# ramkp990/Truth_Recommendation_GNN

Hardware: AMD Instinct MI355X
Metric: edges/s (fwd+bwd) hetero message-passing (higher is better)
Workload: dtype f32; 1 GPU; cfg4: U=9000000 P=1000000 E_engage=200000000 (+reverse), relations=rev_engages+engages, d=h=128, 2-layer hetero-SAGE train step (fwd+loss+bwd+Adam); global_batch=800000000, parallelism=single

## Files before the change

### include/hgnn.h

```cpp
#ifndef HGNN_H_
#define HGNN_H_

#include <stddef.h>
#include <stdint.h>

#ifdef __cplusplus
extern "C" {
#endif

#define HGNN_OK 0
#define HGNN_E_ARG 1001
#define HGNN_E_HIP 1002
#define HGNN_E_WS 1003
#define HGNN_E_UNSUPPORTED 1004

#define HGNN_MEAN 1
#define HGNN_ACCUMULATE 2

#define HGNN_MAX_SEG 6

typedef void* hgnn_stream_t;

int hgnn_version(void);
const char* hgnn_last_error_string(void);
// ... 198 lines not shown

int hgnn_gather_reduce_bf16(const uint16_t* x, int64_t n_x, int32_t d, const int32_t* rowptr,
                            const int32_t* col, int64_t n_rows, const float* edge_w,
                            const float* col_w, const float* row_w, int32_t flags,
                            const int32_t* heavy_rows, const int32_t* heavy_first,
                            int64_t n_heavy, int64_t n_chunks, int32_t chunk, float* slab,
                            float* out, int64_t acc_limit, const int32_t* col_hot,
                            float hot_share, hgnn_stream_t stream);

int hgnn_score_gather2_bf16(const uint16_t* x, int64_t n_x, const uint16_t* rowvec, int32_t d,
                            const int32_t* rowptr, const int32_t* col, const int32_t* rowptr_n,
                            const int32_t* col_n, int64_t n_rows, const float* cscale,
                            float inv_e, const int32_t* heavy_rows, const int32_t* heavy_first,
                            int64_t n_heavy, int64_t n_chunks, int32_t chunk, float* slab,
                            float* out, hgnn_stream_t stream);

int hgnn_edge_score_fwd_bf16(const uint16_t* U, const uint16_t* P, int32_t d, int64_t n_users,
                             int64_t n_posts, const int32_t* rowptr_u, const int32_t* col_u,
                             const int64_t* neg_i64, const int32_t* neg_i32,
                             const uint64_t* d_seed, int64_t n_edges, const float* cscale,
                             float* dU, float* part, float* loss, int32_t* err,
                             hgnn_stream_t stream);

size_t hgnn_sample_ws_bytes(int64_t n_dst);
int hgnn_sample_neighbors(const int32_t* rowptr, const int32_t* col, int64_t n_rows,
                          const int32_t* dst_ids, int64_t n_dst, int32_t fanout, uint64_t seed,
                          int32_t* out_rowptr, int32_t* out_col, void* ws, size_t ws_bytes,
                          hgnn_stream_t stream);
int hgnn_sample_fill(const int32_t* rowptr, const int32_t* col, int64_t n_rows,
                     const int32_t* dst_ids, int64_t n_dst, int32_t fanout, uint64_t seed,
                     const int32_t* out_rowptr, int32_t* out_col, hgnn_stream_t stream);
size_t hgnn_sample_hop_ws_bytes(int64_t n_total_dst);
int hgnn_sample_hop_count(int32_t n_rel, const int32_t* const* rowptrs, const int64_t* n_rows,
                          const int32_t* const* dst_ids, const int64_t* n_dst, int32_t fanout,
                          int32_t* const* out_rowptrs, int32_t* d_totals, void* ws,
                          size_t ws_bytes, hgnn_stream_t stream);
int hgnn_sample_hop_fill(int32_t n_rel, const int32_t* const* rowptrs, const int32_t* const* cols,
                         const int64_t* n_rows, const int32_t* const* dst_ids,
                         const int64_t* n_dst, int32_t fanout, uint64_t seed,
                         const int32_t* const* out_rowptrs, int32_t* const* out_cols,
                         hgnn_stream_t stream);

size_t hgnn_relabel_ws_bytes(int64_t n_prefix, int64_t n_items);
int hgnn_relabel(const int32_t* prefix, int64_t n_prefix, const int32_t* items, int64_t n_items,
                 int32_t* local_out, int32_t* nodes_out, int32_t* d_count, void* ws,
                 size_t ws_bytes, hgnn_stream_t stream);
// ... 98 lines not shown
```

### truth_recommendation_gnn_amd/_native.py

```python
from __future__ import annotations

import ctypes
import os
import pathlib
from typing import Optional, Sequence

import torch

LIB_PATH = pathlib.Path(__file__).resolve().parent / "lib" / "libhgnn.so"
if os.environ.get("HGNN_LIB"):
    LIB_PATH = LIB_PATH.parent / pathlib.Path(os.environ["HGNN_LIB"]).name

HGNN_MEAN = 1
HGNN_ACCUMULATE = 2
MAX_SEG = 6

_c_i32, _c_i64, _c_sz, _p = ctypes.c_int32, ctypes.c_int64, ctypes.c_size_t, ctypes.c_void_p

_SIGS = {
    "hgnn_version": (_c_i32, []),
    "hgnn_last_error_string": (ctypes.c_char_p, []),
    "hgnn_coo_to_csr_ws_bytes": (_c_sz, [_c_i64, _c_i64]),
    "hgnn_coo_to_csr": (_c_i32, [_p, _p, _c_i64, _c_i64, _c_i64, _p, _p, _p, _p, _p, _c_sz, _p]),
    "hgnn_plan_ws_bytes": (_c_sz, [_c_i64]),
# ... 95 lines not shown
    "hgnn_score_topk": (_c_i32, [_p, _p, _c_i64, _p, _c_i64, _c_i32, _c_i32, _p, _p, _p]),
    "hgnn_score_topk_bf16_lds_bytes": (_c_sz, [_c_i32, _c_i32]),
    "hgnn_score_topk_bf16": (_c_i32, [_p, _p, _c_i64, _p, _c_i64, _c_i32, _c_i32, _p, _p, _p]),
    "hgnn_score_topk_excl": (_c_i32, [_p, _p, _c_i64, _p, _c_i64, _c_i32, _c_i32, _p, _p, _p, _p,
                                      _p, _p]),
    "hgnn_score_topk_excl_bf16": (_c_i32, [_p, _p, _c_i64, _p, _c_i64, _c_i32, _c_i32, _p, _p,
                                           _p, _p, _p, _p]),
    "hgnn_topk_finish": (_c_i32, [_p, _p, _c_i64, _c_i32, _c_i64, _c_i32, _p, _p, _p, _p, _p, _p,
                                  _p]),
    "hgnn_edge_score_parts": (_c_i64, [_c_i64]),
    "hgnn_edge_score_fwd": (_c_i32, [_p, _p, _c_i32, _c_i64, _c_i64, _p, _p, _p, _p, _c_i64, _p,
                                     _p, _p, _p, _p, _p, _p, _p, _p, _p]),
    "hgnn_edge_score_fwd_i32": (_c_i32, [_p, _p, _c_i32, _c_i64, _c_i64, _p, _p, _p, _c_i64, _p,
                                         _p, _p, _p, _p, _p]),
    "hgnn_edge_score_fwd_draw": (_c_i32, [_p, _p, _c_i32, _c_i64, _c_i64, _p, _p, _p, _c_i64,
                                          _p, _p, _p, _p, _p, _p]),
    "hgnn_rows_to_bf16": (_c_i32, [_p, _c_i64, _p, _p]),
    "hgnn_gather_reduce_bf16": (_c_i32, [_p, _c_i64, _c_i32, _p, _p, _c_i64, _p, _p, _p, _c_i32,
                                         _p, _p, _c_i64, _c_i64, _c_i32, _p, _p, _c_i64, _p,
                                         ctypes.c_float, _p]),
    "hgnn_score_gather2_bf16": (_c_i32, [_p, _c_i64, _p, _c_i32, _p, _p, _p, _p, _c_i64, _p,
                                         ctypes.c_float, _p, _p, _c_i64, _c_i64, _c_i32, _p, _p,
                                         _p]),
    "hgnn_edge_score_fwd_bf16": (_c_i32, [_p, _p, _c_i32, _c_i64, _c_i64, _p, _p, _p, _p, _p,
                                          _c_i64, _p, _p, _p, _p, _p, _p]),
    "hgnn_uniform_i32": (_c_i32, [_p, _c_i64, _c_i32, _p, _p]),
    "hgnn_scale_unless_one": (_c_i32, [_p, _c_i64, _p, _p]),
    "hgnn_linear_fwd_f32": (_c_i32, [_p, _c_i64, _c_i32, _p, _c_i32, _p, _p, _p]),
    "hgnn_linear_dgrad_f32": (_c_i32, [_p, _c_i64, _c_i32, _p, _c_i32, _p, _p]),
    "hgnn_linear_wgrad_f32": (_c_i32, [_p, _p, _c_i64, _c_i32, _c_i32, _p, _p, _p, _c_sz, _p]),
    "hgnn_hetero_epilogue": (_c_i32, [_c_i32, _p, _p, _c_i64, _c_i32, _p, _p]),
    "hgnn_hetero_epilogue_bwd": (_c_i32, [_c_i32, _p, _c_i64, _c_i32, _p, _p, _p, _p]),
    "hgnn_idmap_capacity": (_c_i64, [_c_i64]),
    "hgnn_idmap_build": (_c_i32, [_p, _p, _p, _c_i64, _p, _c_i64, _p]),
    "hgnn_idmap_lookup": (_c_i32, [_p, _c_i64, _p, _p, _p, _p, _p, _p, _p, _p, _c_i64, _p, _p]),
    "hgnn_compact_rows_ws_bytes": (_c_sz, [_c_i64]),
    "hgnn_compact_rows": (_c_i32, [_p, _c_i32, _c_i64, _p, _p, _c_i32, _p, _p, _c_sz, _p]),
}

_lib: Optional[ctypes.CDLL] = None


class NativeError(RuntimeError):
    pass


# ... 94 lines not shown
```

### truth_recommendation_gnn_amd/build.py

```python
from __future__ import annotations

import concurrent.futures as cf
import hashlib
import json
import os
import pathlib
import subprocess
import sys

PKG = pathlib.Path(__file__).resolve().parent
CSRC = PKG / "csrc"
LIBDIR = PKG / "lib"
LIB = LIBDIR / "libhgnn.so"
INCLUDE = PKG.parent / "include"
HIPCC = os.environ.get("HIPCC", "/opt/rocm/bin/hipcc")
ARCH = "gfx950"
FLAGS = ["-O3", "-std=c++17", "-fPIC", f"--offload-arch={ARCH}", "-Wall",
         "-Wno-unused-result", f"-I{INCLUDE}"]
FILE_FLAGS = {"linear_xs": ["-fno-slp-vectorize"]}


def _sources():
    return sorted(CSRC.glob("*.hip"))


def _digest(extra=(), only=None) -> str:
    h = hashlib.sha256()
    for p in _sources() + sorted(CSRC.glob("*.h")) + [INCLUDE / "hgnn.h"]:
        h.update(p.name.encode())
        h.update(p.read_bytes())
    h.update(" ".join(f for f in FLAGS if not f.startswith("-I")).encode())
    h.update(repr(sorted(FILE_FLAGS.items())).encode())
    if extra:
        h.update(repr((list(extra), sorted(only) if only else None)).encode())
    return h.hexdigest()[:16]


def stamp_path(lib: pathlib.Path) -> pathlib.Path:
    return lib.with_name(lib.name[:-len(".so")] + ".digest")


def check_library(lib: pathlib.Path) -> None:
# ... 51 lines not shown
```

### truth_recommendation_gnn_amd/csrc/gather.hip

```cpp
#include "hgnn_common.h"

#include <stdlib.h>
#include <string.h>

namespace hgnn {

struct GatherArgs {
  const void* x;
  const int32_t* rowptr;
  const int32_t* col;
  const float* edge_w;
  const float* col_w;
  const float* row_w;
  const int32_t* heavy_rows;
  const int32_t* heavy_first;
  float* slab;
  float* out;
  int64_t n_rows;
  int64_t n_heavy;
  int64_t n_items;
  int32_t d;
  int32_t chunk;
  int32_t mean;
  int32_t accumulate;
  int64_t acc_limit;
  const void* rowvec;
  const float* cscale;
  float inv_e;
  int32_t score;
  const int32_t* rowptr2;
  int32_t nt_load;
  int32_t nt_store;
  const int32_t* col2;
  int32_t hot;
  int32_t bf16;
};

constexpr int32_t kHotIdMask = 0x7fffffff;

template <int LPR, int VPL, int W, int UNROLL, bool HAS_W, bool SC, bool HOT, typename XT = float>
__device__ __forceinline__ void segment_sum(const GatherArgs& a, const int32_t* col, int score,
                                            int64_t beg, int64_t end,
                                            const typename Vec<W>::T (&rv)[VPL],
                                            typename Vec<W>::T (&acc)[VPL]) {
  using V = Vec<W>;
  using S = RowSrc<XT, W>;
  constexpr int NS = 64 / LPR;
  const int lane = threadIdx.x & 63;
  const int slot = lane / LPR, sl = lane % LPR;
  const int d = a.d;
  for (int64_t base = beg; base < end; base += 64) {
    const int n = (int)min<int64_t>(64, end - base);
    int cidx = 0;
    float wv = 1.f;
    if (lane < n) {
      cidx = col[base + lane];
      if (HAS_W) {
        wv = a.edge_w ? a.edge_w[base + lane] : 1.f;
        if (a.col_w) wv *= a.col_w[HOT ? cidx & kHotIdMask : cidx];
      }
    }
    for (int j = 0; j < n; j += NS * UNROLL) {
      typename S::Raw v[UNROLL][VPL];
      float we[UNROLL];
#pragma unroll
      for (int u = 0; u < UNROLL; ++u) {
        const int e = j + u * NS + slot;
        const int raw = __shfl(cidx, e & 63, 64);
        const int src = HOT ? raw & kHotIdMask : raw;
// ... 24 lines not shown
        }
      }
#pragma unroll
      for (int u = 0; u < UNROLL; ++u)
#pragma unroll
        for (int q = 0; q < VPL; ++q) {
          if (HAS_W || SC) V::fma(acc[q], we[u], S::widen(v[u][q]));
          else V::add(acc[q], S::widen(v[u][q]));
        }
    }
  }
}

template <int LPR, int VPL, int W>
__device__ __forceinline__ void slot_combine(typename Vec<W>::T (&acc)[VPL]) {
  using V = Vec<W>;
#pragma unroll
  for (int m = LPR; m < 64; m <<= 1)
#pragma unroll
    for (int q = 0; q < VPL; ++q) V::add(acc[q], V::shfl_xor(acc[q], m));
}

template <int LPR, int VPL, int W, int UNROLL, bool HAS_W, bool SC, bool HOT = false,
          typename XT = float>
__device__ __forceinline__ void gather_item(const GatherArgs& a, const int64_t item) {
  using V = Vec<W>;
  using S = RowSrc<XT, W>;
  const int lane = threadIdx.x & 63;
  const int sl = lane % LPR;
  const bool writer = lane < LPR;
  int64_t row, beg, end;
  float* dst;
  bool partial;
  const bool two = SC && a.rowptr2;
  bool own = true;
  if (item < a.n_rows) {
    row = item;
    beg = a.rowptr[row];
    end = a.rowptr[row + 1];
    if (end - beg > a.chunk) {
      if (!two) return;
      own = false;
    }
    dst = a.out + row * a.d;
    partial = false;
  } else {
    const int64_t slot = item - a.n_rows;
    int64_t lo = 0, hi = a.n_heavy;
    while (hi - lo > 1) {
      int64_t mid = (lo + hi) >> 1;
      if (a.heavy_first[mid] <= slot) lo = mid; else hi = mid;
    }
    row = a.heavy_rows[lo];
    const int64_t k = slot - a.heavy_first[lo];
    beg = a.rowptr[row] + k * a.chunk;
    end = min<int64_t>(beg + a.chunk, a.rowptr[row + 1]);
    dst = a.slab + slot * a.d;
    partial = true;
  }
  typename V::T acc[VPL], rv[VPL];
#pragma unroll
  for (int q = 0; q < VPL; ++q) {
    acc[q] = V::zero();
    const int c = (q * LPR + sl) * W;
    rv[q] = (SC && c < a.d)
                ? S::widen(S::load(static_cast<const XT*>(a.rowvec) + row * a.d + c))
                : V::zero();
  }
  if (own)
    segment_sum<LPR, VPL, W, UNROLL, HAS_W, SC, HOT, XT>(a, a.col, a.score, beg, end, rv, acc);
  if (two && !partial)
    segment_sum<LPR, VPL, W, UNROLL, HAS_W, SC, false, XT>(a, a.col2, 2, a.rowptr2[row],
                                                           a.rowptr2[row + 1], rv, acc);
  slot_combine<LPR, VPL, W>(acc);
  if (!writer) return;
  float s = 1.f;
  if (!partial) {
    if (a.row_w) s = a.row_w[row];
    else if (a.mean) s = end > beg ? 1.f / (float)(end - beg) : 0.f;
  }
#pragma unroll
  for (int q = 0; q < VPL; ++q) {
    const int c = (q * LPR + sl) * W;
    if (c < a.d) {
      typename V::T r = acc[q];
      if (!partial) {
        V::scale(r, s);
        if (a.accumulate && (a.acc_limit == 0 || row < a.acc_limit)) V::add(r, V::load(dst + c));
      }
      if (a.nt_store) V::store_nt(dst + c, r);
      else V::store(dst + c, r);
    }
  }
}

template <int LPR, int VPL, int W, int UNROLL, bool HAS_W, bool SC = false, bool HOT = false,
          typename XT = float>
__global__ void __launch_bounds__(256) k_gather(const GatherArgs a) {
  const int64_t item = (int64_t)blockIdx.x * 4 + (threadIdx.x >> 6);
  if (item >= a.n_items) return;
  gather_item<LPR, VPL, W, UNROLL, HAS_W, SC, HOT, XT>(a, item);
}

constexpr int kGatherMultiMax = 8;
struct GatherMulti {
  GatherArgs j[kGatherMultiMax];
  int64_t base[kGatherMultiMax + 1];
  int32_t n;
};

template <int LPR, int VPL, int W, int UNROLL, bool HAS_W>
__global__ void __launch_bounds__(256) k_gather_multi(const GatherMulti m) {
  const int64_t item = (int64_t)blockIdx.x * 4 + __builtin_amdgcn_readfirstlane(threadIdx.x >> 6);
  if (item >= m.base[m.n]) return;
  int j = 0;
  while (j + 1 < m.n && item >= m.base[j + 1]) ++j;
  gather_item<LPR, VPL, W, UNROLL, HAS_W, false>(m.j[j], item - m.base[j]);
}

template <int W>
__global__ void __launch_bounds__(256) k_fixup(const GatherArgs a) {
  using V = Vec<W>;
  __shared__ typename V::T buf[256];
  const int64_t h = blockIdx.x;
// ... 40 lines not shown
    }
    __syncthreads();
  }
}

template <int LPR, int VPL, int W, int UNROLL>
static int launch_gather(const GatherArgs& a, bool has_w, hipStream_t stream) {
  const dim3 grid((unsigned)cdiv(a.n_items, 4)), block(256);
  if (a.score)
    hipLaunchKernelGGL((k_gather<LPR, VPL, W, UNROLL, false, true>), grid, block, 0, stream, a);
  else if (a.hot && has_w)
    hipLaunchKernelGGL((k_gather<LPR, VPL, W, UNROLL, true, false, true>), grid, block, 0, stream,
                       a);
  else if (a.hot)
    hipLaunchKernelGGL((k_gather<LPR, VPL, W, UNROLL, false, false, true>), grid, block, 0,
                       stream, a);
  else if (has_w)
    hipLaunchKernelGGL((k_gather<LPR, VPL, W, UNROLL, true>), grid, block, 0, stream, a);
  else
    hipLaunchKernelGGL((k_gather<LPR, VPL, W, UNROLL, false>), grid, block, 0, stream, a);
  return check_launch("k_gather");
}

static int dispatch_gather(const GatherArgs& a, bool has_w, hipStream_t stream) {
  const int d = a.d;
  if (d % 4 == 0) {
    const int nv = d / 4;
    if (nv <= 4) return launch_gather<4, 1, 4, 4>(a, has_w, stream);
    if (nv <= 8) return launch_gather<8, 1, 4, 4>(a, has_w, stream);
    if (nv <= 16) {
      const dim3 grid((unsigned)cdiv(a.n_items, 4)), block(256);
      if (a.score)
        hipLaunchKernelGGL((k_gather<16, 1, 4, 4, false, true>), grid, block, 0, stream, a);
      else if (a.hot && has_w)
        hipLaunchKernelGGL((k_gather<16, 1, 4, 6, true, false, true>), grid, block, 0, stream, a);
      else if (a.hot)
        hipLaunchKernelGGL((k_gather<16, 1, 4, 8, false, false, true>), grid, block, 0, stream, a);
      else if (has_w)
        hipLaunchKernelGGL((k_gather<16, 1, 4, 6, true>), grid, block, 0, stream, a);
      else
        hipLaunchKernelGGL((k_gather<16, 1, 4, 8, false>), grid, block, 0, stream, a);
      return check_launch("k_gather");
    }
    if (nv <= 32) return launch_gather<32, 1, 4, 4>(a, has_w, stream);
    if (nv <= 64) return launch_gather<64, 1, 4, 4>(a, has_w, stream);
    if (nv <= 128) return launch_gather<64, 2, 4, 2>(a, has_w, stream);
    if (nv <= 256) return launch_gather<64, 4, 4, 2>(a, has_w, stream);
    return fail(HGNN_E_UNSUPPORTED, "gather: d=%d > 1024", d);
// ... 256 lines not shown
  a.rowvec = rowvec; a.cscale = cscale; a.inv_e = inv_e; a.score = mode;
  nt_policy(a, n_x);
  return run_gather(a, as_stream(stream));
}

int hgnn_score_gather2(const float* x, int64_t n_x, const float* rowvec, int32_t d,
                       const int32_t* rowptr, const int32_t* col, const int32_t* rowptr_n,
                       const int32_t* col_n, int64_t n_rows, const float* cscale, float inv_e,
                       const int32_t* heavy_rows, const int32_t* heavy_first, int64_t n_heavy,
                       int64_t n_chunks, int32_t chunk, float* slab, float* out,
                       hgnn_stream_t stream) {
  if (!rowptr_n && n_rows > 0) return fail(HGNN_E_ARG, "score_gather2: rowptr_n is null");
  GatherArgs a{};
  a.x = x; a.rowptr = rowptr; a.col = col;
  a.heavy_rows = heavy_rows; a.heavy_first = heavy_first; a.slab = slab; a.out = out;
  a.n_rows = n_rows; a.n_heavy = n_heavy; a.n_items = n_rows + (n_heavy > 0 ? n_chunks : 0);
  a.d = d; a.chunk = chunk;
  a.rowvec = rowvec; a.cscale = cscale; a.inv_e = inv_e; a.score = 1;
  a.rowptr2 = rowptr_n; a.col2 = col_n;
  nt_policy(a, n_x);
  return run_gather(a, as_stream(stream));
}

int hgnn_score_gather2_bf16(const uint16_t* x, int64_t n_x, const uint16_t* rowvec, int32_t d,
                            const int32_t* rowptr, const int32_t* col, const int32_t* rowptr_n,
                            const int32_t* col_n, int64_t n_rows, const float* cscale,
                            float inv_e, const int32_t* heavy_rows, const int32_t* heavy_first,
                            int64_t n_heavy, int64_t n_chunks, int32_t chunk, float* slab,
                            float* out, hgnn_stream_t stream) {
  if (d > 0 && (d % 8 != 0 || d > 1024))
    return fail(HGNN_E_UNSUPPORTED,
                "score_gather2_bf16: d=%d (bf16 rows need d %% 8 == 0 and d <= 1024)", d);
  if (!rowptr_n && n_rows > 0) return fail(HGNN_E_ARG, "score_gather2_bf16: rowptr_n is null");
  GatherArgs a{};
  a.x = x; a.rowptr = rowptr; a.col = col;
  a.heavy_rows = heavy_rows; a.heavy_first = heavy_first; a.slab = slab; a.out = out;
  a.n_rows = n_rows; a.n_heavy = n_heavy; a.n_items = n_rows + (n_heavy > 0 ? n_chunks : 0);
  a.d = d; a.chunk = chunk;
  a.rowvec = rowvec; a.cscale = cscale; a.inv_e = inv_e; a.score = 1;
  a.rowptr2 = rowptr_n; a.col2 = col_n;
  a.bf16 = 1;
  nt_policy(a, n_x, 2);
  return run_gather(a, as_stream(stream));
}

}
// ... 1 lines not shown
```

### truth_recommendation_gnn_amd/ops.py

```python
from __future__ import annotations

import dataclasses
import os
import weakref
from typing import Dict, List, NamedTuple, Optional, Sequence, Tuple

import torch

from . import _native as N
from .graph import RelationCSR


def _check_f32(t: torch.Tensor, what: str) -> torch.Tensor:
    if t.dtype != torch.float32:
        raise TypeError(f"{what}: hgnn computes in fp32 (the reference dtype); got {t.dtype}")
    return t.contiguous()


ROW_DTYPES = ("fp32", "bf16")


def _row_dtype_value(v: str, what: str) -> str:
    if v not in ROW_DTYPES:
        raise ValueError(f"{what}={v!r}: the row storage is 'fp32' or 'bf16'")
# ... 297 lines not shown
        for i, (x, csr) in enumerate(pairs):
            if i < len(static) and static[i]:
                res[i] = gather_mean(x, csr, static=True,
                                     name=names[i] if i < len(names) else None)
            else:
                rest.append(i)
        if rest:
            for i, o in zip(rest, gather_mean_many([pairs[i] for i in rest])):
                res[i] = o
        return res
    jobs = []
    for x, csr in pairs:
        x = _check_f32(x, "gather_mean")
        if x.shape[0] != csr.n_src:
            raise ValueError(f"x_src has {x.shape[0]} rows, relation expects {csr.n_src}")
        if csr.num_edges and gather_blocks(x, csr.num_edges) > 1:
            return [gather_mean(x, c) for x, c in pairs]
        jobs.append((x, csr.fwd, torch.empty(csr.n_dst, int(x.shape[1]), dtype=torch.float32,
                                             device=x.device)))
    if not _multi_ok(jobs):
        return [gather_mean(x, c) for x, c in pairs]
    _gather_multi(jobs, mean=True, accumulate=False)
    return [o for _, _, o in jobs]


def _table_bytes(x: torch.Tensor) -> int:
    return x.numel() * x.element_size()


def _gather(x, grouped, col_w, csr_mean, out, accumulate, edge_w=None, kind=None, hot=None):
    p = grouped.plan
    dev = out.device
    slab = None
    if p.n_heavy:
        slab = torch.empty(p.n_chunks * out.shape[1], dtype=torch.float32, device=dev)
    flags = (N.HGNN_MEAN if csr_mean else 0) | (N.HGNN_ACCUMULATE if accumulate else 0)
    d = int(out.shape[1])
    weighted = edge_w is not None or col_w is not None
    kind = kind or ("fwd" if csr_mean else "bwd")
    name = f"gather_{kind}[{grouped.n_rows}<-{x.shape[0]}]x{d}"
    E = int(grouped.col.numel())
    rb = _row_bytes(x)
    with _timed(name, gather_bytes(E, grouped.n_rows, d, weighted, rb),
                gather_compulsory_bytes(E, grouped.n_rows, int(x.shape[0]), d, weighted, rb)):
        if x.dtype == torch.bfloat16:
            N.check(N.lib().hgnn_gather_reduce_bf16(
# ... 17 lines not shown
            N.ptr(p.heavy_first), p.n_heavy, p.n_chunks, p.chunk, N.ptr(slab), N.ptr(out),
            N.stream_ptr(dev)), "hgnn_gather_reduce")


def _score_gather(U, P, grouped, mode, cscale, inv_e, out, accumulate, tag):
    p = grouped.plan
    dev = out.device
    d = int(out.shape[1])
    slab = None
    if p.n_heavy:
        slab = torch.empty(p.n_chunks * d, dtype=torch.float32, device=dev)
    E = int(grouped.col.numel())
    nb = gather_bytes(E, grouped.n_rows, d, False) + 4 * grouped.n_rows * d
    cb = (gather_compulsory_bytes(E, grouped.n_rows, int(U.shape[0]), d, False)
          + 4 * grouped.n_rows * d)
    with _timed(f"score_gather_{tag}[{grouped.n_rows}<-{U.shape[0]}]x{d}", nb, cb):
        N.check(N.lib().hgnn_score_gather(
            N.ptr(U), U.shape[0], N.ptr(P), d, N.ptr(grouped.rowptr), N.ptr(grouped.col),
            grouped.n_rows, mode, N.ptr(cscale), inv_e, N.ptr(p.heavy_rows), N.ptr(p.heavy_first),
            p.n_heavy, p.n_chunks, p.chunk, N.ptr(slab), N.ptr(out), 1 if accumulate else 0,
            N.stream_ptr(dev)), "hgnn_score_gather")


def _score_gather2(U, P, pos, negs, cscale, inv_e, out):
    p = pos.plan
    dev = out.device
    d = int(out.shape[1])
    n = pos.n_rows
    slab = None
    if p.n_heavy:
        slab = torch.empty(p.n_chunks * d, dtype=torch.float32, device=dev)
    E = int(pos.col.numel()) + int(negs.col.numel())
    rb = _row_bytes(U)
    nb = gather_bytes(E, n, d, False, rb) + 4 * (n + 1) + n * rb
    cb = gather_compulsory_bytes(E, n, int(U.shape[0]), d, False, rb) + 4 * (n + 1) + n * rb
    with _timed(f"score_gather[{n}<-{U.shape[0]}]x{d}", nb, cb):
        if U.dtype == torch.bfloat16:
            N.check(N.lib().hgnn_score_gather2_bf16(
                N.ptr(U), U.shape[0], N.ptr(P), d, N.ptr(pos.rowptr), N.ptr(pos.col),
                N.ptr(negs.rowptr), N.ptr(negs.col), n, N.ptr(cscale), inv_e,
                N.ptr(p.heavy_rows), N.ptr(p.heavy_first), p.n_heavy, p.n_chunks, p.chunk,
                N.ptr(slab), N.ptr(out), N.stream_ptr(dev)), "hgnn_score_gather2_bf16")
            return
        N.check(N.lib().hgnn_score_gather2(
            N.ptr(U), U.shape[0], N.ptr(P), d, N.ptr(pos.rowptr), N.ptr(pos.col),
            N.ptr(negs.rowptr), N.ptr(negs.col), n, N.ptr(cscale), inv_e, N.ptr(p.heavy_rows),
            N.ptr(p.heavy_first), p.n_heavy, p.n_chunks, p.chunk, N.ptr(slab), N.ptr(out),
            N.stream_ptr(dev)), "hgnn_score_gather2")


def scatter_mean_bwd(grad_aggr: torch.Tensor, csr: RelationCSR,
                     out: Optional[torch.Tensor] = None) -> torch.Tensor:
    grad_aggr = _check_f32(grad_aggr, "scatter_mean_bwd")
    dev = grad_aggr.device
    d = int(grad_aggr.shape[1])
    acc = out is not None
    if out is None:
        out = torch.empty(csr.n_src, d, dtype=torch.float32, device=dev)
    B = gather_blocks(grad_aggr, csr.num_edges) if csr.num_edges else 1
    if B > 1:
        passes, w = csr.blocks("bwd", B)
        E = csr.num_edges
        _gather_blocked(grad_aggr, passes, None, w, out, acc,
                        f"gather_bwd[{csr.n_src}<-{csr.n_dst}]x{d}",
                        gather_bytes(E, csr.n_src, d, True),
# ... 25 lines not shown
    ks = [int(s.shape[1]) for s in segs]
    k = sum(ks)
    if w.shape[1] != k:
        raise ValueError(f"weight has {w.shape[1]} input columns, segments sum to {k}")
    _check_rows(segs, n, what)
    if add is not None and tuple(add.shape) != (n, h):
        raise ValueError(f"{what}: add is {tuple(add.shape)}, expected {(n, h)}")
    if b is not None and b.numel() != h:
        raise ValueError(f"{what}: bias has {b.numel()} entries, expected {h}")
    out = torch.empty(n, h, dtype=torch.float32, device=w.device)
    nb = 4 * n * (k + h + (h if add is not None else 0)) + (16 * n if mask_out is not None else 0)
    return n, h, ks, out, nb, 2 * n * k * h


def linear_fwd(segs: Sequence[torch.Tensor], w: torch.Tensor, b: Optional[torch.Tensor],
               relu: bool, add: Optional[torch.Tensor] = None,
               mask_out: Optional[torch.Tensor] = None) -> torch.Tensor:
    n, h, ks, out, nb, fl = _lin_fwd_job("linear_fwd", segs, w, b, add, mask_out)
    with _timed(f"linear_fwd[{n}x{sum(ks)}->{h}]", nb, flops=fl):
        N.check(N.lib().hgnn_linear_fwd_mask(len(segs), N.ptr_array(segs), N.int_array(ks), n,
                                             N.ptr(w), h, N.ptr(b), N.ptr(add),
                                             1 if relu else 0, N.ptr(out), N.ptr(mask_out),
                                             N.stream_ptr(w.device)), "hgnn_linear_fwd_mask")
    return out


def _lin_bwd_job(what, segs, w, dout, out_act, dxs, need_w, need_b, dz_out=None, mask=None,
                 dx_add=()):
    n = int(segs[0].shape[0])
    h = int(w.shape[0])
    ks = [int(s.shape[1]) for s in segs]
    k = sum(ks)
    if w.shape[1] != k:
        raise ValueError(f"weight has {w.shape[1]} input columns, segments sum to {k}")
    _check_rows(segs, n, what)
    for name, t in (("dout", dout), ("out_act", out_act), ("dz_out", dz_out)):
        if t is not None and tuple(t.shape) != (n, h):
            raise ValueError(f"{what}: {name} is {tuple(t.shape)}, expected {(n, h)}")
    if len(dxs) != len(segs):
        raise ValueError(f"{what}: {len(dxs)} dx buffers for {len(segs)} segments")
    for s_, dx in zip(segs, dxs):
        if dx is not None and tuple(dx.shape) != tuple(s_.shape):
            raise ValueError(f"{what}: dx {tuple(dx.shape)} for a {tuple(s_.shape)} segment")
    if mask is not None and tuple(mask.shape) != (n, 4):
        raise ValueError(f"{what}: ReLU bits are {tuple(mask.shape)}, expected {(n, 4)}")
    dw = torch.empty_like(w) if need_w else None
# ... 44 lines not shown
    out_act: Optional[torch.Tensor]
    dxs: Sequence[Optional[torch.Tensor]]
    need_w: bool
    need_b: bool
    mask: Optional[torch.Tensor]


def linear_fwd_many(jobs) -> List[torch.Tensor]:
    jobs = [FwdJob(*j) for j in jobs]
    if len(jobs) == 1 or len({int(j.w.shape[0]) for j in jobs}) > 1:
        return [linear_fwd(j.segs, j.w, j.b, j.relu, mask_out=j.mask) for j in jobs]
    info = [_lin_fwd_job("linear_fwd_many", j.segs, j.w, j.b, mask_out=j.mask) for j in jobs]
    rows, outs = [i[0] for i in info], [i[3] for i in info]
    ks = [k for i in info for k in i[2]]
    dev, h = jobs[0].w.device, info[0][1]
    with _timed(f"linear_fwd_multi[{'+'.join(str(r) for r in rows)}x{sum(ks) // len(jobs)}->{h}]",
                sum(i[4] for i in info), flops=sum(i[5] for i in info)):
        N.check(N.lib().hgnn_linear_fwd_multi(
            len(jobs), N.int_array([len(j.segs) for j in jobs]),
            N.ptr_array([s_ for j in jobs for s_ in j.segs]), N.int_array(ks), N.i64_array(rows),
            N.ptr_array([j.w for j in jobs]), h, N.ptr_array([j.b for j in jobs]),
            N.int_array([1 if j.relu else 0 for j in jobs]), N.ptr_array(outs),
            N.ptr_array([j.mask for j in jobs]), N.stream_ptr(dev)), "hgnn_linear_fwd_multi")
    return outs


def _linear_bwd_of(j: BwdJob):
    return linear_bwd(j.segs, j.w, j.dout, j.out_act, j.dxs, j.need_w, j.need_b, mask=j.mask)


def linear_bwd_many(jobs):
    jobs = [BwdJob(*j) for j in jobs]
    if len(jobs) == 1 or len({int(j.w.shape[0]) for j in jobs}) > 1:
        return [_linear_bwd_of(j) for j in jobs]
    info = [_lin_bwd_job("linear_bwd_many", j.segs, j.w, j.dout, j.out_act, j.dxs, j.need_w,
                         j.need_b, mask=j.mask) for j in jobs]
    rows, kt = [i[0] for i in info], [sum(i[2]) for i in info]
    dws, dbs = [i[3] for i in info], [i[4] for i in info]
    dev, h = jobs[0].w.device, info[0][1]
    ws = None
    if any(d is not None for d in dws + dbs):
        ws = N.workspace(N.lib().hgnn_linear_bwd_multi_ws_bytes(
            len(jobs), N.i64_array(rows), N.int_array(kt), h), dev)
    with _timed(f"linear_bwd_multi[{'+'.join(str(r) for r in rows)}x{sum(kt) // len(jobs)}->{h}]",
                sum(i[6] for i in info), flops=sum(i[7] for i in info)):
        N.check(N.lib().hgnn_linear_bwd_multi(
# ... 673 lines not shown
    if draw is not None:
        neg = None
    else:
        neg = neg_u_order.contiguous() if neg32 else neg_u_order.to(torch.int64).contiguous()
    return draw, neg32, neg


def presort_negatives(n_users: int, n_posts: int, pos_edges: torch.Tensor, neg_p,
                      neg_order: str) -> PresortedNegatives:
    csr = relation_csr_for_loss(pos_edges, n_users, n_posts)
    neg_u = _negatives_user_order(csr, neg_p, neg_order)
    draw, neg32, neg = _neg_inputs(neg_u)
    dev = csr.fwd.rowptr.device
    err = torch.zeros(2, dtype=torch.int32, device=dev)
    E = csr.num_edges
    rp, us = _sort_negatives(csr, neg_u, draw, neg, neg32, _user_of_pos(csr), E, n_posts, err,
                             dev)
    return PresortedNegatives(csr, neg_p, neg_order, n_posts, rp, us)


def _edge_bce(U, P, csr: RelationCSR, neg_u_order, cscale, check: bool, n_total: int,
              ready=None, on_dP=None, p_chunks=None, presorted=None):
    bf16 = U.dtype == torch.bfloat16
    if bf16:
        if P.dtype != torch.bfloat16:
            raise TypeError("edge_bce_loss: bf16 rows need both tables in bfloat16")
        if ready is not None or on_dP is not None or p_chunks is not None:
            raise ValueError("edge_bce_loss: bf16 rows do not combine with ready / on_dP / "
                             "p_chunks (the sharded step runs on fp32 rows)")
        U, P = U.contiguous(), P.contiguous()
    else:
        U = _check_f32(U, "edge_bce_loss user_emb")
        P = _check_f32(P, "edge_bce_loss post_emb")
    draw = neg_u_order if isinstance(neg_u_order, NegativeDraw) else None
    dev = N.require_device(U, P, draw.seed if draw is not None else neg_u_order)
    lib, s = N.lib(), N.stream_ptr(dev)
    nu, np_, d, E = U.shape[0], P.shape[0], int(U.shape[1]), csr.num_edges
    if P.shape[1] != d or nu != csr.n_src or np_ != csr.n_dst:
        raise ValueError("edge_bce_loss: embedding shapes do not match the positive edges")
    if E == 0:
        if ready is not None:
            ready()
        return (torch.zeros((), dtype=torch.float32, device=dev),
                torch.zeros(U.shape, dtype=torch.float32, device=dev),
                torch.zeros(P.shape, dtype=torch.float32, device=dev))
    ub, pf = csr.bwd, csr.fwd
# ... 11 lines not shown
        neg = None
    else:
        neg = neg_u_order.contiguous() if neg32 else neg_u_order.to(torch.int64).contiguous()
    dP = torch.empty(P.shape, dtype=torch.float32, device=dev)
    if presorted is not None:
        presorted.check_edges(csr, np_)
        rowptr_n, nu_s = presorted.rowptr, presorted.users
    else:
        rowptr_n, nu_s = _sort_negatives(csr, neg_u_order, draw, neg, neg32, uop, E, np_, err,
                                         dev)
    if ready is not None and p_chunks is None:
        ready()
    from .graph import NO_SPLIT, GroupedEdges, Plan
    negs = GroupedEdges(rowptr_n, nu_s, nu_s, Plan(NO_SPLIT, 0, 0, None, None), np_)
    if p_chunks is not None:
        for lo, hi, rdy in p_chunks:
            if rdy is not None:
                rdy()
            if hi > lo:
                ng = GroupedEdges(rowptr_n[lo:hi + 1], nu_s, None,
                                  Plan(NO_SPLIT, 0, 0, None, None), hi - lo)
                _score_gather2(U, P[lo:hi], _row_range(pf, lo, hi), ng, c, inv_e, dP[lo:hi])
    else:
        _score_gather2(U, P, pf, negs, c, inv_e, dP)
    if on_dP is not None:
        on_dP(dP)
    if ready is not None and p_chunks is not None:
        ready()
    rb = _row_bytes(U)
    with _timed(f"edge_score_d{d}", E * (2 * rb + 12) + nu * (rb + 4 * d)):
        if bf16:
            N.check(lib.hgnn_edge_score_fwd_bf16(
                N.ptr(U), N.ptr(P), d, nu, np_, N.ptr(ub.rowptr), N.ptr(ub.col),
                N.ptr(neg) if draw is None and not neg32 else None,
                N.ptr(neg) if draw is None and neg32 else None,
                N.ptr(draw.seed) if draw is not None else None, n_total, N.ptr(c), N.ptr(dU),
                N.ptr(part), N.ptr(loss), N.ptr(err if check else None), s),
                "hgnn_edge_score_fwd_bf16")
        elif draw is not None:
            N.check(lib.hgnn_edge_score_fwd_draw(
                N.ptr(U), N.ptr(P), d, nu, np_, N.ptr(ub.rowptr), N.ptr(ub.col),
                N.ptr(draw.seed), n_total, N.ptr(c), N.ptr(dU), N.ptr(part), N.ptr(loss),
                N.ptr(err if check else None), s), "hgnn_edge_score_fwd_draw")
        elif neg32:
            N.check(lib.hgnn_edge_score_fwd_i32(
                N.ptr(U), N.ptr(P), d, nu, np_, N.ptr(ub.rowptr), N.ptr(ub.col),
                N.ptr(neg), n_total, N.ptr(c), N.ptr(dU), N.ptr(part), N.ptr(loss),
# ... 282 lines not shown
```

Before: 6.296 billion edges/s.

## Zero-pack ReLU user rows to shrink the score-gather traffic

Adds a zero-packed row format, a bitmask plus the non-zero fp32 values in a 128-byte-aligned slot, and a packing kernel that builds it from ReLU-output tables. When the table is at least 1 GiB, d is 64 or 128, and the rows come from a ReLU, the loss's score gather reads the packed rows and expands them in registers using DPP prefix counts of the mask popcounts. The aim is to read fewer bytes per gathered user row in the bandwidth-bound gather over about 400M edges. In exchange it adds a full pass to pack the table, extra memory for the packed copy, and mask decode work per edge.

```diff
diff --git a/include/hgnn.h b/include/hgnn.h
--- a/include/hgnn.h
+++ b/include/hgnn.h
@@ -244,6 +244,20 @@
                              float* dU, float* part, float* loss, int32_t* err,
                              hgnn_stream_t stream);
 
+int64_t hgnn_zpack_slot_bytes(int32_t d);
+
+int32_t hgnn_zpack_policy(int64_t table_bytes, int32_t d, int32_t relu_out);
+
+int hgnn_zpack_rows(const float* x, int64_t n_rows, int32_t d, void* out, int64_t* hist,
+                    hgnn_stream_t stream);
+
+int hgnn_score_gather2_zp(const void* xz, int64_t n_x, const float* rowvec, int32_t d,
+                          const int32_t* rowptr, const int32_t* col, const int32_t* rowptr_n,
+                          const int32_t* col_n, int64_t n_rows, const float* cscale, float inv_e,
+                          const int32_t* heavy_rows, const int32_t* heavy_first, int64_t n_heavy,
+                          int64_t n_chunks, int32_t chunk, float* slab, float* out,
+                          hgnn_stream_t stream);
+
 size_t hgnn_sample_ws_bytes(int64_t n_dst);
 int hgnn_sample_neighbors(const int32_t* rowptr, const int32_t* col, int64_t n_rows,
                           const int32_t* dst_ids, int64_t n_dst, int32_t fanout, uint64_t seed,
diff --git a/truth_recommendation_gnn_amd/_native.py b/truth_recommendation_gnn_amd/_native.py
--- a/truth_recommendation_gnn_amd/_native.py
+++ b/truth_recommendation_gnn_amd/_native.py
@@ -141,6 +141,12 @@
     "hgnn_score_gather2_bf16": (_c_i32, [_p, _c_i64, _p, _c_i32, _p, _p, _p, _p, _c_i64, _p,
                                          ctypes.c_float, _p, _p, _c_i64, _c_i64, _c_i32, _p, _p,
                                          _p]),
+    "hgnn_zpack_slot_bytes": (_c_i64, [_c_i32]),
+    "hgnn_zpack_policy": (_c_i32, [_c_i64, _c_i32, _c_i32]),
+    "hgnn_zpack_rows": (_c_i32, [_p, _c_i64, _c_i32, _p, _p, _p]),
+    "hgnn_score_gather2_zp": (_c_i32, [_p, _c_i64, _p, _c_i32, _p, _p, _p, _p, _c_i64, _p,
+                                       ctypes.c_float, _p, _p, _c_i64, _c_i64, _c_i32, _p, _p,
+                                       _p]),
     "hgnn_edge_score_fwd_bf16": (_c_i32, [_p, _p, _c_i32, _c_i64, _c_i64, _p, _p, _p, _p, _p,
                                           _c_i64, _p, _p, _p, _p, _p, _p]),
     "hgnn_uniform_i32": (_c_i32, [_p, _c_i64, _c_i32, _p, _p]),
diff --git a/truth_recommendation_gnn_amd/build.py b/truth_recommendation_gnn_amd/build.py
--- a/truth_recommendation_gnn_amd/build.py
+++ b/truth_recommendation_gnn_amd/build.py
@@ -17,7 +17,7 @@
 ARCH = "gfx950"
 FLAGS = ["-O3", "-std=c++17", "-fPIC", f"--offload-arch={ARCH}", "-Wall",
          "-Wno-unused-result", f"-I{INCLUDE}"]
-FILE_FLAGS = {"linear_xs": ["-fno-slp-vectorize"]}
+FILE_FLAGS = {"linear_xs": ["-fno-slp-vectorize"], "gather": ["-fno-slp-vectorize"]}
 
 
 def _sources():
diff --git a/truth_recommendation_gnn_amd/csrc/gather.hip b/truth_recommendation_gnn_amd/csrc/gather.hip
--- a/truth_recommendation_gnn_amd/csrc/gather.hip
+++ b/truth_recommendation_gnn_amd/csrc/gather.hip
@@ -1,4 +1,5 @@
 #include "hgnn_common.h"
+#include "zpack.h"
 
 #include <stdlib.h>
 #include <string.h>
@@ -34,17 +35,123 @@
   const int32_t* col2;
   int32_t hot;
   int32_t bf16;
+  int32_t zp;
 };
 
 constexpr int32_t kHotIdMask = 0x7fffffff;
 
-template <int LPR, int VPL, int W, int UNROLL, bool HAS_W, bool SC, bool HOT, typename XT = float>
+typedef uint32_t zp_u4 __attribute__((ext_vector_type(4)));
+typedef zp_u4 zp_u4_a4 __attribute__((aligned(4)));
+template <bool NT>
+__device__ __forceinline__ uint4 zp_load16(const char* p) {
+  zp_u4 v;
+  if constexpr (NT) v = __builtin_nontemporal_load(reinterpret_cast<const zp_u4_a4*>(p));
+  else v = *reinterpret_cast<const zp_u4_a4*>(p);
+  return make_uint4(v.x, v.y, v.z, v.w);
+}
+
+template <int CTRL, int ROWS>
+__device__ __forceinline__ uint32_t dpp_u32(uint32_t x) {
+  return (uint32_t)__builtin_amdgcn_update_dpp(0, (int)x, CTRL, ROWS, 0xF, ROWS == 0xF);
+}
+
+template <int LPR>
+struct ZpMask {
+  static __device__ __forceinline__ uint32_t load(const char* slot, int sl) {
+    return *reinterpret_cast<const uint32_t*>(slot + 4 * zpack::mask_word(sl));
+  }
+  static __device__ __forceinline__ zpack::LaneRead read(uint32_t mw, int sl) {
+    const uint32_t c = zpack::popc(mw);
+    const uint32_t up = dpp_u32<0x118, 0xF>(c);
+    uint32_t below = up;
+    if constexpr (LPR == 32) below += dpp_u32<0x142, 0xA>(c + up);
+    return zpack::lane_read_word(mw, below, sl);
+  }
+};
+
+template <int LPR, int UNROLL, bool NT>
+__device__ __forceinline__ void segment_sum_zp(const GatherArgs& a, const int32_t* col, int score,
+                                               int64_t beg, int64_t end, const float4& rv,
+                                               float4& acc) {
+  using V = Vec<4>;
+  using MK = ZpMask<LPR>;
+  constexpr int NS = 64 / LPR;
+  constexpr int R = NS * UNROLL;
+  static_assert(64 % R == 0, "a round never crosses a 64-edge batch");
+  if (beg >= end) return;
+  const int lane = threadIdx.x & 63;
+  const int slot = lane / LPR, sl = lane % LPR;
+  const char* xb = static_cast<const char*>(a.x);
+  const int64_t S = zpack::slot_bytes(a.d);
+  int cidx = lane < end - beg ? col[beg + lane] : 0;
+  uint32_t m[UNROLL];
+  int src[UNROLL];
+#pragma unroll
+  for (int u = 0; u < UNROLL; ++u) {
+    src[u] = __shfl(cidx, u * NS + slot, 64);
+    m[u] = MK::load(xb + (int64_t)src[u] * S, sl);
+  }
+  for (int64_t base = beg; base < end; base += 64) {
+    const int n = (int)min<int64_t>(64, end - base);
+    const int64_t left = end - base - 64;
+    const int cnext = lane < left ? col[base + 64 + lane] : 0;
+    for (int j = 0; j < n; j += R) {
+      uint4 t[UNROLL];
+      uint32_t nib[UNROLL];
+#pragma unroll
+      for (int u = 0; u < UNROLL; ++u) {
+        const int e = j + u * NS + slot;
+        const zpack::LaneRead L = MK::read(m[u], sl);
+        nib[u] = e < n ? L.nib : 0u;
+        t[u] = zp_load16<NT>(xb + (int64_t)src[u] * S + zpack::value_byte(L.pre));
+      }
+      const bool same = j + R < n;
+      const int csel = same ? cidx : cnext;
+      const int j0 = same ? j + R : 0;
+#pragma unroll
+      for (int u = 0; u < UNROLL; ++u) {
+        src[u] = __shfl(csel, (j0 + u * NS + slot) & 63, 64);
+        m[u] = MK::load(xb + (int64_t)src[u] * S, sl);
+      }
+      float4 v[UNROLL];
+      float we[UNROLL];
+#pragma unroll
+      for (int u = 0; u < UNROLL; ++u) {
+        uint32_t c[4];
+        zpack::expand(t[u].x, t[u].y, t[u].z, t[u].w, nib[u], c);
+        v[u] = make_float4(__uint_as_float(c[0]), __uint_as_float(c[1]), __uint_as_float(c[2]),
+                           __uint_as_float(c[3]));
+      }
+      const float cw = score == 1 ? *a.cscale * a.inv_e : a.inv_e;
+#pragma unroll
+      for (int u = 0; u < UNROLL; ++u) {
+        float sdot = 0.f;
+        sdot += V::dot(rv, v[u]);
+        sdot = slot_sum<LPR>(sdot);
+        const float sg = sigmoid_t(sdot, exp_neg_abs(sdot));
+        we[u] = cw * (score == 1 ? sg - 1.f : sg);
+      }
+#pragma unroll
+      for (int u = 0; u < UNROLL; ++u) V::fma(acc, we[u], v[u]);
+    }
+    cidx = cnext;
+  }
+}
+
+template <int LPR, int VPL, int W, int UNROLL, bool HAS_W, bool SC, bool HOT, typename XT = float,
+          int ZP = 0>
 __device__ __forceinline__ void segment_sum(const GatherArgs& a, const int32_t* col, int score,
                                             int64_t beg, int64_t end,
                                             const typename Vec<W>::T (&rv)[VPL],
                                             typename Vec<W>::T (&acc)[VPL]) {
   using V = Vec<W>;
   using S = RowSrc<XT, W>;
+  if constexpr (ZP != 0) {
+    static_assert(SC && !HAS_W && !HOT && VPL == 1 && W == 4 && sizeof(XT) == 4,
+                  "zero-packed rows: the fp32 score gather at d = 64 / 128");
+    segment_sum_zp<LPR, UNROLL, ZP == 2>(a, col, score, beg, end, rv[0], acc[0]);
+    return;
+  }
   constexpr int NS = 64 / LPR;
   const int lane = threadIdx.x & 63;
   const int slot = lane / LPR, sl = lane % LPR;
@@ -115,7 +222,7 @@
 }
 
 template <int LPR, int VPL, int W, int UNROLL, bool HAS_W, bool SC, bool HOT = false,
-          typename XT = float>
+          typename XT = float, int ZP = 0>
 __device__ __forceinline__ void gather_item(const GatherArgs& a, const int64_t item) {
   using V = Vec<W>;
   using S = RowSrc<XT, W>;
@@ -161,10 +268,11 @@
                 : V::zero();
   }
   if (own)
-    segment_sum<LPR, VPL, W, UNROLL, HAS_W, SC, HOT, XT>(a, a.col, a.score, beg, end, rv, acc);
+    segment_sum<LPR, VPL, W, UNROLL, HAS_W, SC, HOT, XT, ZP>(a, a.col, a.score, beg, end, rv,
+                                                             acc);
   if (two && !partial)
-    segment_sum<LPR, VPL, W, UNROLL, HAS_W, SC, false, XT>(a, a.col2, 2, a.rowptr2[row],
-                                                           a.rowptr2[row + 1], rv, acc);
+    segment_sum<LPR, VPL, W, UNROLL, HAS_W, SC, false, XT, ZP>(a, a.col2, 2, a.rowptr2[row],
+                                                               a.rowptr2[row + 1], rv, acc);
   slot_combine<LPR, VPL, W>(acc);
   if (!writer) return;
   float s = 1.f;
@@ -193,6 +301,14 @@
   const int64_t item = (int64_t)blockIdx.x * 4 + (threadIdx.x >> 6);
   if (item >= a.n_items) return;
   gather_item<LPR, VPL, W, UNROLL, HAS_W, SC, HOT, XT>(a, item);
+}
+
+template <int LPR, int UNROLL, int ZP>
+__global__ void __launch_bounds__(256) __attribute__((amdgpu_waves_per_eu(6)))
+k_gather_zp(const GatherArgs a) {
+  const int64_t item = (int64_t)blockIdx.x * 4 + (threadIdx.x >> 6);
+  if (item >= a.n_items) return;
+  gather_item<LPR, 1, 4, UNROLL, false, true, false, float, ZP>(a, item);
 }
 
 constexpr int kGatherMultiMax = 8;
@@ -279,8 +395,25 @@
   return check_launch("k_gather");
 }
 
+static int dispatch_gather_zp(const GatherArgs& a, hipStream_t stream) {
+  if (!a.score || !zpack::width_ok(a.d))
+    return fail(HGNN_E_UNSUPPORTED, "gather(zero-packed rows): score mode at d = 64 or 128 (d=%d)",
+                a.d);
+  const dim3 grid((unsigned)cdiv(a.n_items, 4)), block(256);
+#define HGNN_GZP(LPR, ZP) \
+  hipLaunchKernelGGL((k_gather_zp<LPR, 4, ZP>), grid, block, 0, stream, a)
+  if (a.d == 64) {
+    if (a.nt_load) HGNN_GZP(16, 2); else HGNN_GZP(16, 1);
+  } else {
+    if (a.nt_load) HGNN_GZP(32, 2); else HGNN_GZP(32, 1);
+  }
+#undef HGNN_GZP
+  return check_launch("k_gather(zp)");
+}
+
 static int dispatch_gather(const GatherArgs& a, bool has_w, hipStream_t stream) {
   const int d = a.d;
+  if (a.zp) return dispatch_gather_zp(a, stream);
   if (d % 4 == 0) {
     const int nv = d / 4;
     if (nv <= 4) return launch_gather<4, 1, 4, 4>(a, has_w, stream);
@@ -583,6 +716,27 @@
   return run_gather(a, as_stream(stream));
 }
 
+int hgnn_score_gather2_zp(const void* xz, int64_t n_x, const float* rowvec, int32_t d,
+                          const int32_t* rowptr, const int32_t* col, const int32_t* rowptr_n,
+                          const int32_t* col_n, int64_t n_rows, const float* cscale, float inv_e,
+                          const int32_t* heavy_rows, const int32_t* heavy_first, int64_t n_heavy,
+                          int64_t n_chunks, int32_t chunk, float* slab, float* out,
+                          hgnn_stream_t stream) {
+  if (!zpack::width_ok(d))
+    return fail(HGNN_E_UNSUPPORTED, "score_gather2_zp: d=%d (zero-packed rows: 64 or 128)", d);
+  if (!rowptr_n && n_rows > 0) return fail(HGNN_E_ARG, "score_gather2_zp: rowptr_n is null");
+  GatherArgs a{};
+  a.x = xz; a.rowptr = rowptr; a.col = col;
+  a.heavy_rows = heavy_rows; a.heavy_first = heavy_first; a.slab = slab; a.out = out;
+  a.n_rows = n_rows; a.n_heavy = n_heavy; a.n_items = n_rows + (n_heavy > 0 ? n_chunks : 0);
+  a.d = d; a.chunk = chunk;
+  a.rowvec = rowvec; a.cscale = cscale; a.inv_e = inv_e; a.score = 1;
+  a.rowptr2 = rowptr_n; a.col2 = col_n;
+  a.zp = 1;
+  nt_policy(a, n_x);
+  return run_gather(a, as_stream(stream));
+}
+
 int hgnn_score_gather2_bf16(const uint16_t* x, int64_t n_x, const uint16_t* rowvec, int32_t d,
                             const int32_t* rowptr, const int32_t* col, const int32_t* rowptr_n,
                             const int32_t* col_n, int64_t n_rows, const float* cscale,
diff --git a/truth_recommendation_gnn_amd/csrc/zpack.h b/truth_recommendation_gnn_amd/csrc/zpack.h
--- /dev/null
+++ b/truth_recommendation_gnn_amd/csrc/zpack.h
@@ -0,0 +1,81 @@
+#pragma once
+#include <stdint.h>
+
+#if defined(__HIPCC__)
+#define HGNN_ZP_HD __host__ __device__
+#else
+#define HGNN_ZP_HD
+#endif
+
+namespace hgnn {
+namespace zpack {
+
+constexpr int kMaskBytes = 16;
+constexpr int kLine = 128;
+constexpr int kHistBins = 6;
+
+HGNN_ZP_HD inline bool width_ok(int d) { return d == 64 || d == 128; }
+
+HGNN_ZP_HD inline int64_t slot_bytes(int d) {
+  return width_ok(d) ? (int64_t)kLine * ((kMaskBytes + 4 * d + 12 + kLine - 1) / kLine) : 0;
+}
+
+HGNN_ZP_HD inline uint32_t popc(uint32_t x) { return (uint32_t)__builtin_popcount(x); }
+
+HGNN_ZP_HD inline int row_lines(int nnz) { return (kMaskBytes + 4 * nnz + kLine - 1) / kLine; }
+
+HGNN_ZP_HD inline uint32_t nibble_of(uint32_t x0, uint32_t x1, uint32_t x2, uint32_t x3) {
+  return (x0 ? 1u : 0u) | (x1 ? 2u : 0u) | (x2 ? 4u : 0u) | (x3 ? 8u : 0u);
+}
+
+HGNN_ZP_HD inline int mask_word(int sl) { return sl >> 3; }
+HGNN_ZP_HD inline int mask_shift(int sl) { return (sl & 7) * 4; }
+
+struct LaneRead {
+  uint32_t pre;
+  uint32_t nib;
+};
+
+HGNN_ZP_HD inline LaneRead lane_read(uint32_t m0, uint32_t m1, uint32_t m2, uint32_t m3, int sl) {
+  const int w = mask_word(sl), b = mask_shift(sl);
+  const uint32_t low = (1u << b) - 1u, all = ~0u;
+  const uint32_t k0 = w > 0 ? all : low;
+  const uint32_t k1 = w > 1 ? all : (w == 1 ? low : 0u);
+  const uint32_t k2 = w > 2 ? all : (w == 2 ? low : 0u);
+  const uint32_t k3 = w == 3 ? low : 0u;
+  const uint32_t lo = (w & 2) ? m2 : m0, hi = (w & 2) ? m3 : m1;
+  const uint32_t mw = (w & 1) ? hi : lo;
+  LaneRead r;
+  r.pre = popc(m0 & k0) + popc(m1 & k1) + popc(m2 & k2) + popc(m3 & k3);
+  r.nib = (mw >> b) & 15u;
+  return r;
+}
+
+HGNN_ZP_HD inline LaneRead lane_read_word(uint32_t mw, uint32_t below, int sl) {
+  const int b = mask_shift(sl);
+  LaneRead r;
+  r.pre = below + popc(mw & ((1u << b) - 1u));
+  r.nib = (mw >> b) & 15u;
+  return r;
+}
+
+HGNN_ZP_HD inline int value_byte(uint32_t k) { return kMaskBytes + 4 * (int)k; }
+
+HGNN_ZP_HD inline uint32_t value_index(uint32_t pre, uint32_t nib, int j) {
+  return pre + popc(nib & ((1u << j) - 1u));
+}
+
+HGNN_ZP_HD inline void expand(uint32_t t0, uint32_t t1, uint32_t t2, uint32_t t3, uint32_t nib,
+                              uint32_t (&v)[4]) {
+  const bool b0 = nib & 1u, b1 = nib & 2u, b2 = nib & 4u, b3 = nib & 8u;
+  v[0] = b0 ? t0 : 0u;
+  const uint32_t p0 = b0 ? t1 : t0, p1 = b0 ? t2 : t1, p2 = b0 ? t3 : t2;
+  v[1] = b1 ? p0 : 0u;
+  const uint32_t q0 = b1 ? p1 : p0, q1 = b1 ? p2 : p1;
+  v[2] = b2 ? q0 : 0u;
+  const uint32_t r0 = b2 ? q1 : q0;
+  v[3] = b3 ? r0 : 0u;
+}
+
+}
+}
diff --git a/truth_recommendation_gnn_amd/csrc/zpack.hip b/truth_recommendation_gnn_amd/csrc/zpack.hip
--- /dev/null
+++ b/truth_recommendation_gnn_amd/csrc/zpack.hip
@@ -0,0 +1,96 @@
+#include "hgnn_common.h"
+#include "zpack.h"
+
+#include <stdlib.h>
+#include <string.h>
+
+namespace hgnn {
+
+template <int LPR>
+__global__ void __launch_bounds__(256) k_zpack(const float* __restrict__ x, const int64_t n_rows,
+                                               unsigned char* __restrict__ out,
+                                               unsigned long long* __restrict__ hist) {
+  constexpr int D = LPR * 4;
+  constexpr int RPB = 256 / LPR;
+  __shared__ unsigned int h[zpack::kHistBins];
+  if (hist) {
+    if (threadIdx.x < zpack::kHistBins) h[threadIdx.x] = 0;
+    __syncthreads();
+  }
+  const int sl = threadIdx.x % LPR;
+  const int64_t r = (int64_t)blockIdx.x * RPB + threadIdx.x / LPR;
+  const bool live = r < n_rows;
+  uint4 xv = make_uint4(0u, 0u, 0u, 0u);
+  if (live) xv = *reinterpret_cast<const uint4*>(x + r * D + 4 * sl);
+  const uint32_t nib = zpack::nibble_of(xv.x, xv.y, xv.z, xv.w);
+  uint32_t w = nib << zpack::mask_shift(sl);
+  w |= __shfl_xor(w, 1, 64);
+  w |= __shfl_xor(w, 2, 64);
+  w |= __shfl_xor(w, 4, 64);
+  const int g0 = (threadIdx.x & 63) - sl;
+  const uint32_t m0 = __shfl(w, g0, 64), m1 = __shfl(w, g0 + 8, 64);
+  const uint32_t m2 = LPR > 16 ? __shfl(w, g0 + 16, 64) : 0u;
+  const uint32_t m3 = LPR > 16 ? __shfl(w, g0 + 24, 64) : 0u;
+  const zpack::LaneRead L = zpack::lane_read(m0, m1, m2, m3, sl);
+  if (live) {
+    unsigned char* slot = out + r * zpack::slot_bytes(D);
+    if (sl == 0) *reinterpret_cast<uint4*>(slot) = make_uint4(m0, m1, m2, m3);
+    const uint32_t xs[4] = {xv.x, xv.y, xv.z, xv.w};
+#pragma unroll
+    for (int j = 0; j < 4; ++j)
+      if (nib & (1u << j))
+        *reinterpret_cast<uint32_t*>(slot + zpack::value_byte(zpack::value_index(L.pre, nib, j))) =
+            xs[j];
+  }
+  if (hist) {
+    if (live && sl == 0) {
+      const int nnz = (int)(zpack::popc(m0) + zpack::popc(m1) + zpack::popc(m2) + zpack::popc(m3));
+      atomicAdd(&h[zpack::row_lines(nnz)], 1u);
+    }
+    __syncthreads();
+    if (threadIdx.x < zpack::kHistBins && h[threadIdx.x])
+      atomicAdd(hist + threadIdx.x, (unsigned long long)h[threadIdx.x]);
+  }
+}
+
+constexpr int64_t kZpackBytes = int64_t(1) << 30;
+static bool zpack_policy(int64_t table_bytes, int d, bool relu_out) {
+  if (!zpack::width_ok(d)) return false;
+  const char* e = getenv("HGNN_ZPACK");
+  if (e && !strcmp(e, "0")) return false;
+  if (e && !strcmp(e, "1")) return true;
+  return relu_out && table_bytes >= kZpackBytes;
+}
+
+}
+
+using namespace hgnn;
+
+extern "C" {
+
+int64_t hgnn_zpack_slot_bytes(int32_t d) { return zpack::slot_bytes(d); }
+
+int32_t hgnn_zpack_policy(int64_t table_bytes, int32_t d, int32_t relu_out) {
+  return zpack_policy(table_bytes, d, relu_out != 0) ? 1 : 0;
+}
+
+int hgnn_zpack_rows(const float* x, int64_t n_rows, int32_t d, void* out, int64_t* hist,
+                    hgnn_stream_t stream) {
+  if (!zpack::width_ok(d)) return fail(HGNN_E_UNSUPPORTED, "zpack_rows: d=%d (64 or 128)", d);
+  if (n_rows < 0) return fail(HGNN_E_ARG, "zpack_rows: n_rows=%lld", (long long)n_rows);
+  if (n_rows == 0) return HGNN_OK;
+  if (!x || !out) return fail(HGNN_E_ARG, "zpack_rows: null x/out");
+  unsigned char* o = static_cast<unsigned char*>(out);
+  unsigned long long* hg = reinterpret_cast<unsigned long long*>(hist);
+  const dim3 block(256);
+  if (d == 64) {
+    const dim3 grid((unsigned)cdiv(n_rows, 256 / 16));
+    hipLaunchKernelGGL(k_zpack<16>, grid, block, 0, as_stream(stream), x, n_rows, o, hg);
+  } else {
+    const dim3 grid((unsigned)cdiv(n_rows, 256 / 32));
+    hipLaunchKernelGGL(k_zpack<32>, grid, block, 0, as_stream(stream), x, n_rows, o, hg);
+  }
+  return check_launch("k_zpack");
+}
+
+}
diff --git a/truth_recommendation_gnn_amd/ops.py b/truth_recommendation_gnn_amd/ops.py
--- a/truth_recommendation_gnn_amd/ops.py
+++ b/truth_recommendation_gnn_amd/ops.py
@@ -343,6 +343,27 @@
         return [gather_mean(x, c) for x, c in pairs]
     _gather_multi(jobs, mean=True, accumulate=False)
     return [o for _, _, o in jobs]
+
+
+RELU_OUT = "_hgnn_relu_out"
+
+
+def zpack_on(x: torch.Tensor, relu_out: bool) -> bool:
+    return bool(N.lib().hgnn_zpack_policy(_table_bytes(x), int(x.shape[1]), 1 if relu_out else 0))
+
+
+def zpack_rows(x: torch.Tensor, hist: Optional[torch.Tensor] = None) -> torch.Tensor:
+    x = _check_f32(x, "zpack_rows")
+    dev = N.require_device(x)
+    n, d = int(x.shape[0]), int(x.shape[1])
+    slot = int(N.lib().hgnn_zpack_slot_bytes(d))
+    if slot == 0:
+        raise ValueError(f"zpack_rows: d={d}; zero-packed rows are 64 or 128 wide")
+    out = torch.empty(n * slot, dtype=torch.uint8, device=dev)
+    with _timed(f"zpack[{n}]x{d}", n * (4 * d + 16 + 4 * d)):
+        N.check(N.lib().hgnn_zpack_rows(N.ptr(x), n, d, N.ptr(out), N.ptr(hist),
+                                        N.stream_ptr(dev)), "hgnn_zpack_rows")
+    return out
 
 
 def _table_bytes(x: torch.Tensor) -> int:
@@ -406,7 +427,7 @@
             N.stream_ptr(dev)), "hgnn_score_gather")
 
 
-def _score_gather2(U, P, pos, negs, cscale, inv_e, out):
+def _score_gather2(U, P, pos, negs, cscale, inv_e, out, Uz=None):
     p = pos.plan
     dev = out.device
     d = int(out.shape[1])
@@ -425,6 +446,13 @@
                 N.ptr(negs.rowptr), N.ptr(negs.col), n, N.ptr(cscale), inv_e,
                 N.ptr(p.heavy_rows), N.ptr(p.heavy_first), p.n_heavy, p.n_chunks, p.chunk,
                 N.ptr(slab), N.ptr(out), N.stream_ptr(dev)), "hgnn_score_gather2_bf16")
+            return
+        if Uz is not None:
+            N.check(N.lib().hgnn_score_gather2_zp(
+                N.ptr(Uz), U.shape[0], N.ptr(P), d, N.ptr(pos.rowptr), N.ptr(pos.col),
+                N.ptr(negs.rowptr), N.ptr(negs.col), n, N.ptr(cscale), inv_e,
+                N.ptr(p.heavy_rows), N.ptr(p.heavy_first), p.n_heavy, p.n_chunks, p.chunk,
+                N.ptr(slab), N.ptr(out), N.stream_ptr(dev)), "hgnn_score_gather2_zp")
             return
         N.check(N.lib().hgnn_score_gather2(
             N.ptr(U), U.shape[0], N.ptr(P), d, N.ptr(pos.rowptr), N.ptr(pos.col),
@@ -496,6 +524,8 @@
                                              N.ptr(w), h, N.ptr(b), N.ptr(add),
                                              1 if relu else 0, N.ptr(out), N.ptr(mask_out),
                                              N.stream_ptr(w.device)), "hgnn_linear_fwd_mask")
+    if relu:
+        setattr(out, RELU_OUT, True)
     return out
 
 
@@ -586,6 +616,9 @@
             N.ptr_array([j.w for j in jobs]), h, N.ptr_array([j.b for j in jobs]),
             N.int_array([1 if j.relu else 0 for j in jobs]), N.ptr_array(outs),
             N.ptr_array([j.mask for j in jobs]), N.stream_ptr(dev)), "hgnn_linear_fwd_multi")
+    for j, o in zip(jobs, outs):
+        if j.relu:
+            setattr(o, RELU_OUT, True)
     return outs
 
 
@@ -1305,6 +1338,7 @@
 def _edge_bce(U, P, csr: RelationCSR, neg_u_order, cscale, check: bool, n_total: int,
               ready=None, on_dP=None, p_chunks=None, presorted=None):
     bf16 = U.dtype == torch.bfloat16
+    relu_out = bool(getattr(U, RELU_OUT, False))
     if bf16:
         if P.dtype != torch.bfloat16:
             raise TypeError("edge_bce_loss: bf16 rows need both tables in bfloat16")
@@ -1362,7 +1396,11 @@
                                   Plan(NO_SPLIT, 0, 0, None, None), hi - lo)
                 _score_gather2(U, P[lo:hi], _row_range(pf, lo, hi), ng, c, inv_e, dP[lo:hi])
     else:
-        _score_gather2(U, P, pf, negs, c, inv_e, dP)
+        Uz = None
+        if not bf16 and ready is None and zpack_on(U, relu_out):
+            Uz = zpack_rows(U)
+        _score_gather2(U, P, pf, negs, c, inv_e, dP, Uz)
+        del Uz
     if on_dP is not None:
         on_dP(dP)
     if ready is not None and p_chunks is not None:
```

Measured after the change: 6.464 billion edges/s (median of 6 runs). +2.7%, better.
